# furiosa-ai/eta-inversion

Measured on AMD Instinct MI355X. Metric: images/sec SD1.5 512^2 50-step etainv+ptp, higher is better.
Workload: dtype bf16; 1 GPU; etainv+ptp, SD1.5-shaped UNet (seeded synthetic weights), 512x512 (64x64 latents), 50 DDIM steps, 32 image pairs per GPU per step, eta [[0.6, 0], [1, 0.7]], n=10 noise candidates, cfg 7.5/1; images_per_gpu=32, unet_sample_forwards_per_image_reference=300

## Files before the change

### eta-inversion_amd/csrc/common.h

```cpp
#pragma once
#include <hip/hip_runtime.h>
#include <stdint.h>
#include <stdio.h>
#include <stdlib.h>
#include <string>

#include "../../include/etainv.h"

namespace etainv {

typedef _Float16 f16;
typedef __bf16 bf16;
typedef float f32x4 __attribute__((ext_vector_type(4)));
typedef float f32x2 __attribute__((ext_vector_type(2)));
typedef float f32x16 __attribute__((ext_vector_type(16)));
typedef _Float16 f16x8 __attribute__((ext_vector_type(8)));
typedef _Float16 f16x4 __attribute__((ext_vector_type(4)));
typedef __bf16 bf16x8 __attribute__((ext_vector_type(8)));
typedef __bf16 bf16x4 __attribute__((ext_vector_type(4)));
typedef unsigned int u32x4 __attribute__((ext_vector_type(4)));
typedef unsigned int u32x2 __attribute__((ext_vector_type(2)));

void set_error(const std::string& msg);
#define ETAINV_FAIL(msg)                                                        \
// ... 16 lines not shown
    if (_e != hipSuccess) ETAINV_FAIL(std::string("launch: ") + hipGetErrorString(_e)); \
  } while (0)

template <typename T> __device__ __forceinline__ float to_f32(T v);
template <> __device__ __forceinline__ float to_f32<float>(float v) { return v; }
template <> __device__ __forceinline__ float to_f32<f16>(f16 v) { return (float)v; }
template <> __device__ __forceinline__ float to_f32<bf16>(bf16 v) { return (float)v; }
template <typename T> __device__ __forceinline__ T from_f32(float v);
template <> __device__ __forceinline__ float from_f32<float>(float v) { return v; }
template <> __device__ __forceinline__ f16 from_f32<f16>(float v) { return (f16)v; }
template <> __device__ __forceinline__ bf16 from_f32<bf16>(float v) { return (bf16)v; }

__device__ __forceinline__ float wave_sum(float v) {
#pragma unroll
  for (int o = 32; o > 0; o >>= 1) v += __shfl_xor(v, o, 64);
  return v;
}
__device__ __forceinline__ float wave_max(float v) {
#pragma unroll
  for (int o = 32; o > 0; o >>= 1) v = fmaxf(v, __shfl_xor(v, o, 64));
  return v;
}

__device__ __forceinline__ float silu_f(float x) { return x / (1.0f + __expf(-x)); }
typedef float gelu_f32x2 __attribute__((ext_vector_type(2)));
__device__ __forceinline__ gelu_f32x2 gelu_pair(gelu_f32x2 x) {
  gelu_f32x2 ax;
  ax[0] = fminf(fabsf(x[0]) * 0.70710678118654752f, 4.3f);
  ax[1] = fminf(fabsf(x[1]) * 0.70710678118654752f, 4.3f);
  gelu_f32x2 p = ax * 0.000100211372f + (-0.000461519738f);
  p = p * ax + (-0.00230234699f);
  p = p * ax + 0.0294526188f;
  p = p * ax + (-0.148963716f);
  p = p * ax + (-0.918328635f);
  p = p * ax + (-1.62791373f);
  const gelu_f32x2 t = p * ax;
  gelu_f32x2 e;
  e[0] = __builtin_amdgcn_exp2f(t[0]);
  e[1] = __builtin_amdgcn_exp2f(t[1]);
  const gelu_f32x2 er = 1.0f - e;
  gelu_f32x2 s;
  s[0] = copysignf(er[0], x[0]);
  s[1] = copysignf(er[1], x[1]);
  const gelu_f32x2 h = x * 0.5f;
  return h * s + h;
}
__device__ __forceinline__ float gelu_erf_f(float x) {
// ... 63 lines not shown
```

### eta-inversion_amd/csrc/kernels.h

```cpp
#pragma once
#include "common.h"

namespace etainv {

struct IGemmParams {
  const void* a1 = nullptr;
  const void* a2 = nullptr;
  const void* w = nullptr;
  const float* bias = nullptr;
  const float* rowvec = nullptr;
  int rowvec_stride = 0;
  int out_f32 = 0;
  int out_nchw = 0;
  int pad0 = 0;
  int out_io_dtype = 0;
  const void* residual = nullptr;
  void* out = nullptr;
  const void* zeros = nullptr;
  int debug = 0;
  int hm_heads = 0, hm_dim = 0, hm_tokens = 0, hm_magic = 0;
  unsigned long* stamps = nullptr;
  int M = 0, N = 0;
  int c1 = 0, c2 = 0;
  int H = 1, W = 1;
// ... 101 lines not shown
  float* maps_acc = nullptr;
  int xcd_gx = 0;
};
inline void cross_params_from_ctrl(CrossParams& cp, const etainv_attn_ctrl* ctrl) {
  if (!ctrl || (ctrl->mode != ETAINV_ATTN_PTP && ctrl->mode != ETAINV_ATTN_STORE)) return;
  const bool ptp = ctrl->mode == ETAINV_ATTN_PTP;
  cp.n_img = ctrl->n_img;
  cp.layout = ptp ? (ctrl->src_exit_block ? 3 : 2) : 1;
  cp.first_row = ptp ? ctrl->first_row : 0;
  if (ptp && (ctrl->mapper || ctrl->replace_mat)) {
    cp.edit = 1;
    cp.mapper = ctrl->mapper;
    cp.alphas = ctrl->alphas;
    cp.replace_mat = ctrl->replace_mat;
    cp.equalizer = ctrl->equalizer;
    cp.cross_alpha = ctrl->cross_alpha;
  }
}
int launch_cross_attention_p(const void* q, const void* kv, void* out, int b, int d, const CrossParams& p, int dtype, hipStream_t s);

int launch_im2col_in(const void* latent, int io_dtype, int n_lat, int rows, int L, void* out, int dtype, hipStream_t s);
int launch_time_embedding(const int64_t* t_host, int rows, int dim, void* out, int dtype, hipStream_t s);
int launch_silu(const void* x, void* out, int64_t n, int dtype, hipStream_t s);
enum PackMode { PK_PLAIN = 0, PK_CONV = 1, PK_GEGLU = 2, PK_CONV_IN_GEMM = 5 };
int launch_pack_ups4(const float* src, void* dst, int cout, int cin, int dtype, hipStream_t s);
int launch_pack_weight(const float* src, void* dst, int64_t rows, int64_t cols, int mode, int taps, int dtype, hipStream_t s, float scale = 1.0f,
                       const float* colscale = nullptr);
int launch_ln_fold(const float* w_src, const float* gamma, const float* beta, const float* bias_packed, int64_t rows, int64_t cols, int mode, float scale,
                   void* w_dst, float* s_dst, float* c_dst, int dtype, hipStream_t s);
int launch_cast_f32(const void* src, int src_dtype, void* dst, int dst_dtype, int64_t n, hipStream_t s);
int launch_rows_broadcast(void* x, int rows, int n_src, int64_t row_elems, int dtype, hipStream_t s);

int launch_prox_guidance(const float* eps_u, const float* eps_c, float g, int mode, int use_rank, int rank_lo, float rank_w, float thr_fixed,
                         float* eps_out, const float* x, float a_from, float a_to, float* x_out, float* thr_out, int n_groups, int rows_per_group,
                         int l, hipStream_t s);

int launch_image_metrics(const float* pred, const float* target, int b, int h, int w, float lo, float hi, int mask, float* out, void* workspace,
                         int64_t workspace_bytes, hipStream_t s);

int launch_word_maps(const float* maps_acc, int n_layers, int n_img_cap, int rows_per_img, int row_sel, int heads, int res, int L,
                     int n_img, const int32_t* tokens, int n_tok, int steps_done, float* out, int accumulate, float scale,
                     hipStream_t s, unsigned layer_mask = ~0u);
int launch_local_blend(const float* maps_acc, int n_layers, int n_img_cap, int heads, int res, int L, float* x, int n_img,
                       const float* blend_alpha, float thres, hipStream_t s);

}
// ... 1 lines not shown
```

### eta-inversion_amd/csrc/misc.hip

```cpp
#include <algorithm>

#include "common.h"
#include "kernels.h"

namespace etainv {

template <typename T, typename TIO>
__global__ void im2col_in_kernel(const TIO* __restrict__ x, int n_lat, int L, int rows, T* __restrict__ out) {
  const int LL = L * L;
  const int64_t i = (int64_t)blockIdx.x * blockDim.x + threadIdx.x;
  if (i >= (int64_t)rows * LL) return;
  const int row = (int)(i / LL), pix = (int)(i - (int64_t)row * LL);
  const int oy = pix / L, ox = pix - oy * L;
  const TIO* xb = x + (int64_t)(row % n_lat) * 4 * LL;
  T v[64];
#pragma unroll
  for (int k = 0; k < 64; ++k) v[k] = (T)0.f;
#pragma unroll
  for (int t = 0; t < 9; ++t) {
    const int iy = oy + t / 3 - 1, ix = ox + t % 3 - 1;
    if (iy >= 0 && iy < L && ix >= 0 && ix < L) {
#pragma unroll
      for (int ci = 0; ci < 4; ++ci) v[t * 4 + ci] = from_f32<T>(to_f32(xb[(int64_t)ci * LL + iy * L + ix]));
    }
  }
  u32x4* o = reinterpret_cast<u32x4*>(out + i * 64);
#pragma unroll
  for (int q = 0; q < (int)(64 * sizeof(T) / 16); ++q) o[q] = reinterpret_cast<u32x4*>(v)[q];
}

struct TimeVec { float t[64]; };
template <typename T>
__global__ void time_embedding_kernel(TimeVec tv, int uniform, int row0, int rows, int dim, T* __restrict__ out) {
  const int i = blockIdx.x * blockDim.x + threadIdx.x;
  if (i >= rows * dim) return;
  const int r = i / dim, c = i - r * dim, half = dim / 2;
  const int k = c < half ? c : c - half;
  const float freq = expf(-9.210340371976184f * (float)k / (float)half);
  const float a = tv.t[uniform ? 0 : r] * freq;
  out[(int64_t)row0 * dim + i] = from_f32<T>(c < half ? cosf(a) : sinf(a));
}

template <typename T>
__global__ void silu_kernel(const T* x, T* out, int64_t n) {
  int64_t i = (int64_t)blockIdx.x * blockDim.x + threadIdx.x;
  if (i < n) out[i] = from_f32<T>(silu_f(to_f32(x[i])));
}

template <typename TD>
__global__ void pack_weight_kernel(const float* __restrict__ src, TD* __restrict__ dst, int64_t rows, int64_t cols, int mode, int taps, float scale,
                                   const float* __restrict__ colscale) {
  const int64_t i = (int64_t)blockIdx.x * blockDim.x + threadIdx.x;
  if (mode == 5) {
    if (i >= rows * 64) return;
    const int64_t o = i / 64, k = i - o * 64, tap = k / 4, ci = k - tap * 4;
    dst[i] = from_f32<TD>(k < 36 ? src[o * 36 + ci * 9 + tap] : 0.f);
    return;
  }
  if (i >= rows * cols) return;
  int64_t s = i;
  if (mode == 1) {
    const int64_t o = i / cols, r = i - o * cols, cin = cols / taps;
    const int64_t t = r / cin, ci = r - t * cin;
    s = o * cols + ci * taps + t;
  } else if (mode == 2) {
    const int64_t p = i / cols, c = i - p * cols;
    const int64_t blk = p / 64, within = p % 64;
    const int64_t logical = within < 32 ? blk * 32 + within : rows / 2 + blk * 32 + within - 32;
    s = logical * cols + c;
// ... 47 lines not shown
}

int launch_time_embedding(const int64_t* t_host, int rows, int dim, void* out, int dtype, hipStream_t s) {
  ETAINV_CHECK(t_host && out && dim % 2 == 0 && rows > 0, "bad arguments");
  bool uniform = true;
  for (int i = 1; i < rows; ++i) uniform = uniform && t_host[i] == t_host[0];
  TimeVec tv;
  if (uniform) {
    tv.t[0] = (float)t_host[0];
    ETAINV_DISPATCH_DTYPE(dtype, T, hipLaunchKernelGGL(time_embedding_kernel<T>, dim3(cdiv(rows * dim, 256)), dim3(256), 0, s, tv, 1, 0, rows, dim, (T*)out));
  } else {
    for (int r0 = 0; r0 < rows; r0 += 64) {
      const int n = std::min(64, rows - r0);
      for (int i = 0; i < n; ++i) tv.t[i] = (float)t_host[r0 + i];
      ETAINV_DISPATCH_DTYPE(dtype, T, hipLaunchKernelGGL(time_embedding_kernel<T>, dim3(cdiv(n * dim, 256)), dim3(256), 0, s, tv, 0, r0, n, dim, (T*)out));
    }
  }
  ETAINV_LAUNCH_CHECK();
  return 0;
}

int launch_silu(const void* x, void* out, int64_t n, int dtype, hipStream_t s) {
  ETAINV_DISPATCH_DTYPE(dtype, T, hipLaunchKernelGGL(silu_kernel<T>, dim3(cdiv(n, 256)), dim3(256), 0, s, (const T*)x, (T*)out, n));
  ETAINV_LAUNCH_CHECK();
  return 0;
}

template <typename TD>
__global__ void pack_ups4_kernel(const float* __restrict__ src, TD* __restrict__ dst, int cout, int cin) {
  const int64_t total = (int64_t)16 * cout * cin;
  const int64_t i = (int64_t)blockIdx.x * 256 + threadIdx.x;
  if (i >= total) return;
  const int c = (int)(i % cin);
  const int t = (int)((i / cin) & 3);
  const int n = (int)((i / ((int64_t)4 * cin)) % cout);
  const int ph = (int)(i / ((int64_t)4 * cin * cout));
  const int py = ph >> 1, px = ph & 1, ty = t >> 1, tx = t & 1;
  const int ky0 = py == 0 ? (ty == 0 ? 0 : 1) : (ty == 0 ? 0 : 2), ky1 = py == 0 ? (ty == 0 ? 0 : 2) : (ty == 0 ? 1 : 2);
  const int kx0 = px == 0 ? (tx == 0 ? 0 : 1) : (tx == 0 ? 0 : 2), kx1 = px == 0 ? (tx == 0 ? 0 : 2) : (tx == 0 ? 1 : 2);
  const float* w = src + ((int64_t)n * cin + c) * 9;
  float v = 0.f;
  for (int ky = ky0; ky <= ky1; ++ky)
    for (int kx = kx0; kx <= kx1; ++kx) v += w[ky * 3 + kx];
  dst[i] = from_f32<TD>(v);
}
int launch_pack_ups4(const float* src, void* dst, int cout, int cin, int dtype, hipStream_t s) {
// ... 96 lines not shown
```

### eta-inversion_amd/csrc/norm.hip

```cpp
#include "common.h"
#include "kernels.h"

namespace etainv {

constexpr int GN_MAX_VEC_PER_LANE = 5;
#ifndef GN_UNROLL
#define GN_UNROLL 4
#endif

template <typename T> struct Vec8;
template <> struct Vec8<f16> { typedef f16x8 type; };
template <> struct Vec8<bf16> { typedef bf16x8 type; };

template <typename T>
__device__ __forceinline__ void load8(const T* p, float (&v)[8]) {
  typename Vec8<T>::type r = *reinterpret_cast<const typename Vec8<T>::type*>(p);
#pragma unroll
  for (int j = 0; j < 8; ++j) v[j] = (float)r[j];
}
template <typename T>
__device__ __forceinline__ void store8(T* p, const float (&v)[8]) {
  typename Vec8<T>::type r;
#pragma unroll
  for (int j = 0; j < 8; ++j) r[j] = (T)v[j];
// ... 55 lines not shown
    for (int o = 1; o < 8; o <<= 1) {
      a += __shfl_xor(a, o);
      c += __shfl_xor(c, o);
    }
    if (g < groups && sub == 0) {
      float* p = partial + (((int64_t)b * chunks + blockIdx.x) * groups + g) * 2;
      p[0] = a;
      p[1] = c;
    }
  } else if (threadIdx.x < groups) {
    const int g = threadIdx.x;
    float a = 0.f, c = 0.f;
    for (int w = 0; w < 4; ++w)
      for (int ch = g * cpg; ch < (g + 1) * cpg; ++ch) {
        a += sm[(w * C + ch) * 2 + 0];
        c += sm[(w * C + ch) * 2 + 1];
      }
    float* p = partial + (((int64_t)b * chunks + blockIdx.x) * groups + g) * 2;
    p[0] = a;
    p[1] = c;
  }
}

template <typename T, int VPL>
__global__ void __launch_bounds__(256) gn_apply_kernel(const T* __restrict__ x1, const T* __restrict__ x2, int c1, int c2, int hw,
                                                       int groups, const float* __restrict__ partial, int chunks_st, float count,
                                                       float eps, const float* __restrict__ gamma, const float* __restrict__ beta,
                                                       int silu, T* __restrict__ out) {
  const int C = c1 + c2, nvec = C >> 3, nv1 = c1 >> 3, cpg = C / groups;
  const int b = blockIdx.y, chunks = gridDim.x;
  const int per = (hw + chunks - 1) / chunks;
  const int beg = blockIdx.x * per, end = min(hw, beg + per);
  const int lane = threadIdx.x & 63, wid = threadIdx.x >> 6;
  __shared__ double s_red[8][64][2];
  __shared__ float st[64 * 2];
  const bool pre_scsh = chunks_st == 0 && gamma == nullptr;
  if (pre_scsh) {
  } else if (chunks_st == 0) {
    if (threadIdx.x < groups) {
      st[threadIdx.x * 2 + 0] = partial[((int64_t)b * groups + threadIdx.x) * 2 + 0];
      st[threadIdx.x * 2 + 1] = partial[((int64_t)b * groups + threadIdx.x) * 2 + 1];
    }
    __syncthreads();
  } else {
    const int NS = groups <= 32 ? 8 : 4;
    const int g = groups <= 32 ? (threadIdx.x & 31) : lane, slice = groups <= 32 ? (threadIdx.x >> 5) : wid;
    double a = 0.0, c = 0.0;
    if (g < groups) {
      f32x2 v[8];
#pragma unroll
      for (int u = 0; u < 8; ++u) {
        const int k = slice + u * NS;
        v[u] = (f32x2){0.f, 0.f};
        if (k < chunks_st) v[u] = *reinterpret_cast<const f32x2*>(partial + (((int64_t)b * chunks_st + k) * groups + g) * 2);
      }
#pragma unroll
      for (int u = 0; u < 8; ++u) { a += v[u][0]; c += v[u][1]; }
      for (int k = slice + 8 * NS; k < chunks_st; k += NS) {
        const float* p = partial + (((int64_t)b * chunks_st + k) * groups + g) * 2;
        a += p[0];
        c += p[1];
      }
      s_red[slice][g][0] = a;
      s_red[slice][g][1] = c;
    }
    __syncthreads();
    if (threadIdx.x < groups) {
      const int g = threadIdx.x;
      double sa = 0.0, sq = 0.0;
      for (int w = 0; w < NS; ++w) { sa += s_red[w][g][0]; sq += s_red[w][g][1]; }
      const double mean = sa / count;
      double var = sq / count - mean * mean;
      if (var < 0.0) var = 0.0;
      st[g * 2 + 0] = (float)mean;
      st[g * 2 + 1] = (float)(1.0 / sqrt(var + (double)eps));
    }
    __syncthreads();
  }
  if constexpr (VPL == 0) {
    constexpr int R = 5;
    const int G = 320 / nvec;
    float sc[R][8], sh[R][8];
    int poff[R], voff[R];
    bool second[R];
#pragma unroll
    for (int r = 0; r < R; ++r) {
      const int idx = lane + 64 * r;
      const int px = idx / nvec, v = idx - px * nvec;
      poff[r] = px;
      second[r] = v >= nv1;
      voff[r] = (second[r] ? v - nv1 : v) * 8;
      if (pre_scsh) {
        const float* ps = partial + ((int64_t)b * 2) * C + v * 8;
        *reinterpret_cast<f32x4*>(&sc[r][0]) = *reinterpret_cast<const f32x4*>(ps);
        *reinterpret_cast<f32x4*>(&sc[r][4]) = *reinterpret_cast<const f32x4*>(ps + 4);
        *reinterpret_cast<f32x4*>(&sh[r][0]) = *reinterpret_cast<const f32x4*>(ps + C);
        *reinterpret_cast<f32x4*>(&sh[r][4]) = *reinterpret_cast<const f32x4*>(ps + C + 4);
        continue;
      }
      int g = (v * 8) / cpg, rem = v * 8 - g * cpg;
#pragma unroll
      for (int j = 0; j < 8; ++j) {
        const int ch = v * 8 + j;
        const float a = st[g * 2 + 1] * gamma[ch];
        sc[r][j] = a;
        sh[r][j] = beta[ch] - st[g * 2] * a;
        if (++rem == cpg) { rem = 0; ++g; }
      }
    }
    for (int pix0 = beg + wid * G; pix0 < end; pix0 += 4 * G) {
      float t[R][8];
      bool ok[R];
#pragma unroll
      for (int r = 0; r < R; ++r) {
        const int pix = pix0 + poff[r];
        ok[r] = pix < end;
        const int64_t row = (int64_t)b * hw + (ok[r] ? pix : beg);
        if (second[r]) load8(x2 + row * c2 + voff[r], t[r]);
        else load8(x1 + row * c1 + voff[r], t[r]);
      }
#pragma unroll
      for (int r = 0; r < R; ++r) {
#pragma unroll
        for (int j = 0; j < 8; ++j) {
          const float y = t[r][j] * sc[r][j] + sh[r][j];
          t[r][j] = silu ? silu_f(y) : y;
        }
        const int pix = pix0 + poff[r];
        if (ok[r]) store8(out + ((int64_t)b * hw + pix) * C + (second[r] ? nv1 * 8 : 0) + voff[r], t[r]);
      }
    }
    return;
  }
  constexpr int VP = VPL > 0 ? VPL : 1;
  float sc[VP][8], sh[VP][8];
#pragma unroll
  for (int i = 0; i < VP; ++i) {
    const int v = lane + 64 * i;
    if (v < nvec) {
      if (pre_scsh) {
        const float* ps = partial + ((int64_t)b * 2) * C + v * 8;
        *reinterpret_cast<f32x4*>(&sc[i][0]) = *reinterpret_cast<const f32x4*>(ps);
        *reinterpret_cast<f32x4*>(&sc[i][4]) = *reinterpret_cast<const f32x4*>(ps + 4);
        *reinterpret_cast<f32x4*>(&sh[i][0]) = *reinterpret_cast<const f32x4*>(ps + C);
        *reinterpret_cast<f32x4*>(&sh[i][4]) = *reinterpret_cast<const f32x4*>(ps + C + 4);
        continue;
      }
      int g = (v * 8) / cpg, rem = v * 8 - g * cpg;
#pragma unroll
      for (int j = 0; j < 8; ++j) {
        const int ch = v * 8 + j;
        const float a = st[g * 2 + 1] * gamma[ch];
        sc[i][j] = a;
        sh[i][j] = beta[ch] - st[g * 2] * a;
        if (++rem == cpg) { rem = 0; ++g; }
      }
    }
  }
#pragma unroll(VP <= 2 ? GN_UNROLL : 1)
  for (int pix = beg + wid; pix < end; pix += 4) {
    const int64_t row = (int64_t)b * hw + pix;
#pragma unroll
    for (int i = 0; i < VP; ++i) {
      const int v = lane + 64 * i;
      if (v < nvec) {
        float t[8];
        if (v < nv1) load8(x1 + row * c1 + v * 8, t);
        else load8(x2 + row * c2 + (v - nv1) * 8, t);
#pragma unroll
        for (int j = 0; j < 8; ++j) {
          const float y = t[j] * sc[i][j] + sh[i][j];
          t[j] = silu ? silu_f(y) : y;
        }
        store8(out + row * C + v * 8, t);
      }
    }
  }
}

template <typename T>
__global__ void __launch_bounds__(256) layernorm_kernel(const T* __restrict__ x, const float* __restrict__ gamma,
                                                        const float* __restrict__ beta, T* __restrict__ out, int rows, int C,
                                                        float eps) {
  const int lane = threadIdx.x & 63;
  const int row = blockIdx.x * 4 + (threadIdx.x >> 6);
  if (row >= rows) return;
  const int nvec = C >> 3;
  float t[3][8];
  float sum = 0.f;
#pragma unroll
  for (int i = 0; i < 3; ++i) {
    const int v = lane + 64 * i;
    if (v < nvec) {
      load8(x + (int64_t)row * C + v * 8, t[i]);
#pragma unroll
      for (int j = 0; j < 8; ++j) sum += t[i][j];
    }
  }
  const float mean = wave_sum(sum) / (float)C;
// ... 94 lines not shown
  }
#pragma unroll
  for (int o = 1; o < 64; o <<= 1) {
    a += __shfl_xor(a, o);
    q += __shfl_xor(q, o);
  }
  const double count = (double)hw * (double)cpg;
  const double mean = a / count;
  double var = q / count - mean * mean;
  if (var < 0.0) var = 0.0;
  const float fmean = (float)mean, frstd = (float)(1.0 / sqrt(var + (double)eps));
  if (lane == 0) {
    final_stats[((int64_t)b * groups + g) * 2 + 0] = fmean;
    final_stats[((int64_t)b * groups + g) * 2 + 1] = frstd;
  }
  if (scsh)
    for (int ch = lo + lane; ch < hi; ch += 64) {
      const float sc = frstd * gamma[ch];
      scsh[((int64_t)b * 2 + 0) * C + ch] = sc;
      scsh[((int64_t)b * 2 + 1) * C + ch] = beta[ch] - fmean * sc;
    }
}

static inline int gn_apply_blocks() {
  static const int n = env_int("ETAINV_GN_APPLY_BLOCKS", 2048);
  return n;
}

static inline int gn_apply_mode(int C) {
  static const bool no_flat = env_on("ETAINV_GN_NOFLAT");
  const int nvec = C >> 3;
  if (!no_flat && (nvec == 40 || nvec == 80)) return 0;
  return (nvec + 63) / 64;
}

int launch_groupnorm(const void* x1, const void* x2, int c1, int c2, const float* gamma, const float* beta, void* out, int b,
                     int hw, int groups, float eps, int silu, float* scratch, int dtype, hipStream_t s) {
  if (dtype == ETAINV_F32) return launch_groupnorm_f32(x1, x2, c1, c2, gamma, beta, out, b, hw, groups, eps, silu, scratch, s);
  const int C = c1 + c2;
  ETAINV_CHECK(x1 && gamma && beta && out && scratch, "null pointer");
  ETAINV_CHECK(c1 % 8 == 0 && c2 % 8 == 0 && C % groups == 0 && groups <= 64, "channel layout");
  ETAINV_CHECK((C >> 3) <= 64 * GN_MAX_VEC_PER_LANE, "C too large");
  ETAINV_CHECK(c2 == 0 || x2, "second source missing");
  int chunks = std::min(GN_MAX_CHUNKS, std::max(1, std::min(hw / 8, 1024 / std::max(1, b))));
  float* partial = scratch;
  const size_t lds = (size_t)4 * C * 2 * sizeof(float);
  const int chunks_apply = std::max(1, std::min(hw / 4, std::max(chunks, gn_apply_blocks() / std::max(1, b))));
  ProfScope prof(PROF_GROUPNORM, 2.0 * 2.0 * (double)b * hw * C, s);
  const int vpl = ((C >> 3) + 63) / 64;
#define ETAINV_GN_LAUNCH(VPL_)                                                                                                             \
  {                                                                                                                                        \
    allow_dynamic_lds<&gn_stats_kernel<T, VPL_>>(4 * 64 * VPL_ * 8 * 2 * 4);                                                               \
    hipLaunchKernelGGL((gn_stats_kernel<T, VPL_>), dim3(chunks, b), dim3(256), lds, s, (const T*)x1, (const T*)x2, c1, c2, hw, groups, partial); \
  }
#define ETAINV_GN_APPLY(VPL_)                                                                                                              \
  hipLaunchKernelGGL((gn_apply_kernel<T, VPL_>), dim3(chunks_apply, b), dim3(256), 0, s, (const T*)x1, (const T*)x2, c1, c2, hw, groups,     \
                     (const float*)partial, chunks, (float)hw * (float)(C / groups), eps, gamma, beta, silu, (T*)out);
  ETAINV_DISPATCH_HALF(dtype, T, switch (vpl) {
    case 1: ETAINV_GN_LAUNCH(1) break;
    case 2: ETAINV_GN_LAUNCH(2) break;
    case 3: ETAINV_GN_LAUNCH(3) break;
    case 4: ETAINV_GN_LAUNCH(4) break;
    default: ETAINV_GN_LAUNCH(5) break;
  } switch (gn_apply_mode(C)) {
    case 0: ETAINV_GN_APPLY(0) break;
    case 1: ETAINV_GN_APPLY(1) break;
    case 2: ETAINV_GN_APPLY(2) break;
    case 3: ETAINV_GN_APPLY(3) break;
    case 4: ETAINV_GN_APPLY(4) break;
    default: ETAINV_GN_APPLY(5) break;
  });
#undef ETAINV_GN_APPLY
#undef ETAINV_GN_LAUNCH
  ETAINV_LAUNCH_CHECK();
  return 0;
}

int launch_gn_finalize(int c1, int c2, const float* part1, int wm1, const float* part2, int wm2, int b, int hw, int groups, float eps, float* final_stats,
                       hipStream_t s, const float* gamma, const float* beta, float* scsh) {
  ETAINV_CHECK(part1 && final_stats && (c1 + c2) % groups == 0 && groups <= 32, "bad arguments");
  ETAINV_CHECK(wm1 > 0 && hw % wm1 == 0 && (c2 == 0 || (part2 && wm2 > 0 && hw % wm2 == 0)), "row blocks must tile an image");
  ProfScope prof(PROF_GROUPNORM, 0.0, s);
  hipLaunchKernelGGL(gn_finalize_kernel, dim3((groups + 3) / 4, b), dim3(256), 0, s, part1, wm1, c1, part2, wm2, c2, hw, groups, eps, final_stats, gamma, beta,
                     scsh);
  ETAINV_LAUNCH_CHECK();
  return 0;
}

int launch_groupnorm_pre(const void* x1, const void* x2, int c1, int c2, const float* part1, int wm1, const float* part2, int wm2, const float* gamma,
                         const float* beta, void* out, int b, int hw, int groups, float eps, int silu, float* final_stats, int dtype, hipStream_t s) {
  const int C = c1 + c2;
  ETAINV_CHECK(x1 && gamma && beta && out && part1 && final_stats, "null pointer");
  ETAINV_CHECK(c1 % 8 == 0 && c2 % 8 == 0 && C % groups == 0 && groups <= 32, "channel layout");
  ETAINV_CHECK((C >> 3) <= 64 * GN_MAX_VEC_PER_LANE, "C too large");
  ETAINV_CHECK(c2 == 0 || (x2 && part2), "second source missing");
  ETAINV_CHECK(wm1 > 0 && hw % wm1 == 0 && (c2 == 0 || (wm2 > 0 && hw % wm2 == 0)), "row blocks must tile an image");
  ProfScope prof(PROF_GROUPNORM, 2.0 * 2.0 * (double)b * hw * C, s);
  prof_pause(true);
  float* scsh = final_stats + (int64_t)b * groups * 2;
  const int rc = launch_gn_finalize(c1, c2, part1, wm1, part2, wm2, b, hw, groups, eps, final_stats, s, gamma, beta, scsh);
  prof_pause(false);
  if (rc) return 1;
  const int chunks_apply = std::max(1, std::min(hw / 4, std::max(std::min(GN_MAX_CHUNKS, std::max(1, std::min(hw / 8, 1024 / std::max(1, b)))), gn_apply_blocks() / std::max(1, b))));
#define ETAINV_GN_APPLY(VPL_)                                                                                                              \
  hipLaunchKernelGGL((gn_apply_kernel<T, VPL_>), dim3(chunks_apply, b), dim3(256), 0, s, (const T*)x1, (const T*)x2, c1, c2, hw, groups,     \
                     (const float*)scsh, 0, (float)hw * (float)(C / groups), eps, (const float*)nullptr, (const float*)nullptr, silu, (T*)out);
  ETAINV_DISPATCH_HALF(dtype, T, switch (gn_apply_mode(C)) {
    case 0: ETAINV_GN_APPLY(0) break;
    case 1: ETAINV_GN_APPLY(1) break;
    case 2: ETAINV_GN_APPLY(2) break;
    case 3: ETAINV_GN_APPLY(3) break;
    case 4: ETAINV_GN_APPLY(4) break;
    default: ETAINV_GN_APPLY(5) break;
  });
#undef ETAINV_GN_APPLY
  ETAINV_LAUNCH_CHECK();
  return 0;
}

int launch_layernorm(const void* x, const float* gamma, const float* beta, void* out, int rows, int c, float eps, int dtype,
                     hipStream_t s) {
  if (dtype == ETAINV_F32) return launch_layernorm_f32(x, gamma, beta, out, rows, c, eps, s);
  ETAINV_CHECK(x && gamma && beta && out, "null pointer");
  ETAINV_CHECK(c % 8 == 0 && (c >> 3) <= 192, "LayerNorm width must be a multiple of 8 and <= 1536");
  ProfScope prof(PROF_LAYERNORM, 2.0 * 2.0 * (double)rows * c, s);
  ETAINV_DISPATCH_HALF(dtype, T,
                       hipLaunchKernelGGL(layernorm_kernel<T>, dim3(cdiv(rows, 4)), dim3(256), 0, s, (const T*)x, gamma, beta,
                                          (T*)out, rows, c, eps));
  ETAINV_LAUNCH_CHECK();
  return 0;
}

int launch_row_stats(const void* x, float* stat, int rows, int c, float eps, int dtype, hipStream_t s) {
  ETAINV_CHECK(x && stat, "null pointer");
  ETAINV_CHECK(c % 8 == 0 && (c >> 3) <= 192, "row width must be a multiple of 8 and <= 1536");
  ProfScope prof(PROF_LAYERNORM, 2.0 * (double)rows * c, s);
  ETAINV_DISPATCH_HALF(dtype, T, hipLaunchKernelGGL(row_stats_kernel<T>, dim3(cdiv(rows, 4)), dim3(256), 0, s, (const T*)x, stat, rows, c, eps));
// ... 14 lines not shown
```

### eta-inversion_amd/csrc/ops_capi.cpp

```cpp
#include <cmath>

#include "common.h"
#include "kernels.h"

using namespace etainv;

extern "C" int etainv_op_gemm(const void* a, const void* w, const void* bias, const void* residual, void* out, int m, int n, int k,
                              int geglu, int dtype, void* stream) {
  IGemmParams p = igemm_linear(a, w, (const float*)bias, out, m, n, k);
  p.residual = residual;
  p.geglu = geglu;
  return launch_igemm(p, dtype, (hipStream_t)stream);
}

extern "C" int etainv_op_gemm_ln(const void* a, const void* w_folded, const float* c_vec, const float* s_vec, const float* stat,
                                 const void* residual, void* out, float* stat_out, int* stat_p_out, int m, int n, int k, int geglu,
                                 int dtype, void* stream) {
  IGemmParams p = igemm_linear(a, w_folded, c_vec, out, m, n, k);
  p.residual = residual;
  p.geglu = geglu;
  if (stat) {
    p.ln_stat = stat;
    p.ln_s = s_vec;
  }
// ... 150 lines not shown
}

extern "C" int etainv_op_gemm_per_image(const void* a, const void* wb, const float* cb, const void* residual, void* out, int b, int hw, int n, int k,
                                        int dtype, void* stream) {
  ETAINV_CHECK(b > 0 && hw > 0, "bad sizes");
  IGemmParams p = igemm_linear(a, wb, cb, out, b * hw, n, k);
  p.residual = residual;
  p.rows_per_batch = hw;
  p.w_batch_stride = (int64_t)n * k;
  p.bias_batch_stride = n;
  return launch_igemm(p, dtype, (hipStream_t)stream);
}

extern "C" int etainv_op_time_embedding(const int64_t* t_host, int rows, int dim, void* out, int dtype, void* stream) {
  return launch_time_embedding(t_host, rows, dim, out, dtype, (hipStream_t)stream);
}

extern "C" int etainv_op_silu(const void* x, void* out, int64_t n, int dtype, void* stream) {
  ETAINV_CHECK(x && out && n >= 0, "null pointer or negative size");
  if (n == 0) return 0;
  return launch_silu(x, out, n, dtype, (hipStream_t)stream);
}

extern "C" int etainv_op_cast(const void* src, int src_dtype, void* dst, int dst_dtype, int64_t n, void* stream) {
  ETAINV_CHECK(src && dst && n >= 0, "null pointer or negative size");
  if (n == 0) return 0;
  return launch_cast_f32(src, src_dtype, dst, dst_dtype, n, (hipStream_t)stream);
}

extern "C" int etainv_op_im2col_in(const void* latent, int io_dtype, int n_lat, int rows, int l, void* out, int dtype, void* stream) {
  ETAINV_CHECK(l > 0, "bad sizes");
  return launch_im2col_in(latent, io_dtype, n_lat, rows, l, out, dtype, (hipStream_t)stream);
}

extern "C" int etainv_op_pack_weight(const float* src, void* dst, int64_t rows, int64_t cols, int mode, int taps, float scale, const float* colscale,
                                     int dtype, void* stream) {
  return launch_pack_weight(src, dst, rows, cols, mode, taps, dtype, (hipStream_t)stream, scale, colscale);
}

extern "C" int etainv_op_word_maps_ex(const float* maps_acc, int n_layers, int n_img_cap, int heads, int res, int L, int n_img, const int32_t* tokens,
                                      int n_tok, int steps_done, int row_sel, unsigned layer_mask, float* out, int accumulate, float scale, void* stream) {
  ETAINV_CHECK(row_sel == 0 || row_sel == 1, "row_sel: 0 = source cond row, 1 = target cond row");
  ETAINV_CHECK(n_img <= n_img_cap && heads > 0 && res > 0 && L > 0, "bad sizes");
  return launch_word_maps(maps_acc, n_layers, n_img_cap, 2, row_sel, heads, res, L, n_img, tokens, n_tok, steps_done, out, accumulate, scale,
                          (hipStream_t)stream, layer_mask);
}
// ... 13 lines not shown
```

### eta-inversion_amd/etainv/_capi.py

```python
import ctypes as C
import os
from pathlib import Path

F32, F16, BF16 = 0, 1, 2
ATTN_PLAIN, ATTN_STORE, ATTN_PTP, ATTN_MASA, ATTN_PNP = 0, 1, 2, 3, 4

_LIB_PATH = Path(__file__).resolve().parent / "lib" / "libetainv_hip.so"


class EtainvError(RuntimeError):
    pass


class EngineConfig(C.Structure):
    _fields_ = [("compute_dtype", C.c_int), ("max_unet_batch", C.c_int), ("latent_size", C.c_int), ("max_img", C.c_int),
                ("reserved", C.c_int * 4)]


class AttnCtrl(C.Structure):
    _fields_ = [("mode", C.c_int), ("n_img", C.c_int), ("store_maps", C.c_int),
                ("mapper", C.c_void_p), ("alphas", C.c_void_p), ("replace_mat", C.c_void_p), ("equalizer", C.c_void_p),
                ("cross_alpha", C.c_void_p),
                ("self_replace_active", C.c_int), ("self_max_tokens", C.c_int),
                ("masa_active", C.c_int), ("masa_first_block", C.c_int), ("first_row", C.c_int), ("src_exit_block", C.c_int), ("pnp_qk_active", C.c_int), ("pnp_conv_active", C.c_int)]
# ... 51 lines not shown
    "etainv_op_conv3x3_gnstat": [_p, _p, _p, _p, _p, _p, _p, C.POINTER(_i), _i, _i, _i, _i, _i, _i, _p],
    "etainv_op_groupnorm_pre": [_p, _p, _i, _i, _p, _i, _p, _i, _p, _p, _p, _i, _i, _i, _f, _i, _p, _i, _p],
    "etainv_op_ln_fold": [_p, _p, _p, _p, _i, _i, _i, _f, _p, _p, _p, _i, _p],
    "etainv_op_row_stats": [_p, _p, _i, _i, _f, _i, _p],
    "etainv_op_ln_finalize": [_p, _i, _i, _f, _p, _i, _p],
    "etainv_op_pack_ups4": [_p, _p, _i, _i, _i, _p],
    "etainv_op_conv3x3": [_p, _p, _i, _i, _p, _p, _p, _p, _p, _i, _i, _i, _i, _i, _i, _i, _i, _p],
    "etainv_op_conv3x3_ex": [_p, _p, _p, _p, _p, _i, _i, _i, _i, _i, _i, _i, _i, _i, _i, _i, _p],
    "etainv_op_im2col3x3": [_p, _i, _i, _i, _i, _i, _p, _p, _i, _p],
    "etainv_op_row_softmax": [_p, _i, _i, _f, _i, _p],
    "etainv_op_quick_gelu": [_p, _p, _i64, _i, _p],
    "etainv_op_embed": [_p, _p, _p, _i, _i, _i, _p, _i, _p],
    "etainv_op_causal_attention": [_p, _p, _i, _i, _i, _i, _i, _p],
    "etainv_op_groupnorm": [_p, _p, _i, _i, _p, _p, _p, _i, _i, _i, _f, _i, _p, _i, _p],
    "etainv_op_layernorm": [_p, _p, _p, _p, _i, _i, _f, _i, _p],
    "etainv_op_self_attention": [_p, _p, _i, _i, _i, _i, _i, _i, _i, _p],
    "etainv_op_self_attention_ex": [_p, _p, _i, _i, _i, _i, _i, _i, _i, _i, _i, _i, _p],
    "etainv_op_cross_attention": [_p, _p, _p, _i, _i, _i, _i, _i, C.POINTER(AttnCtrl), _i, _i, _p, _i, _p],
    "etainv_op_word_maps": [_p, _i, _i, _i, _i, _i, _i, _p, _i, _i, _p, _i, _f, _p],
    "etainv_op_local_blend": [_p, _i, _i, _i, _i, _i, _p, _i, _p, _f, _p],
    "etainv_op_word_maps_ex": [_p, _i, _i, _i, _i, _i, _i, _p, _i, _i, _i, C.c_uint, _p, _i, _f, _p],
    "etainv_op_time_embedding": [C.POINTER(_i64), _i, _i, _p, _i, _p],
    "etainv_op_silu": [_p, _p, _i64, _i, _p],
    "etainv_op_cast": [_p, _i, _p, _i, _i64, _p],
    "etainv_op_im2col_in": [_p, _i, _i, _i, _i, _p, _i, _p],
    "etainv_op_pack_weight": [_p, _p, _i64, _i64, _i, _i, _f, _p, _i, _p],
    "etainv_op_gemm_f32out": [_p, _p, _p, _p, _i, _i, _i, _i, _p],
    "etainv_op_conv3x3_rv": [_p, _p, _i, _i, _p, _p, _p, _i, _p, _p, _i, _i, _i, _i, _i, _i, _i, _i, _p],
    "etainv_op_gn_fold": [_p, _p, _p, _p, _p, _i, _i, _i, _i, _p, _p, _i, _p],
    "etainv_op_gemm_per_image": [_p, _p, _p, _p, _p, _i, _i, _i, _i, _i, _p],
    "etainv_op_rows_broadcast": [_p, _i, _i, _i64, _i, _p],
}
_RESTYPES = {"etainv_last_error": C.c_char_p, "etainv_engine_workspace_bytes": _i64, "etainv_image_metrics_workspace_bytes": _i64, "etainv_engine_weight_bytes": _i64}

_lib = None


def lib_path() -> Path:
    return Path(os.environ.get("ETAINV_LIB", _LIB_PATH))


def load():
    global _lib
    if _lib is None:
        path = lib_path()
        if not path.exists():
# ... 31 lines not shown
```

### include/etainv.h

```cpp
#ifndef ETAINV_H
#define ETAINV_H
#include <stdint.h>
#ifdef __cplusplus
extern "C" {
#endif

#define ETAINV_ABI_VERSION 1
#define ETAINV_MAX_WORDS 77

enum etainv_dtype { ETAINV_F32 = 0, ETAINV_F16 = 1, ETAINV_BF16 = 2 };

int etainv_abi_version(void);
const char* etainv_last_error(void);


int etainv_cfg_combine(const void* eps_u, const void* eps_c, float g, void* out, int64_t n,
                       int io_dtype, void* stream);

int etainv_ddim_step(const void* x, const void* eps, float a_from, float a_to, void* out, int64_t n,
                     int io_dtype, void* stream);

int etainv_ddim_eta_step(const void* x, const void* eps, float eta, const void* eta_mask, int n_mask, const void* noise,
                         float a_t, float a_p, float var, int rows, int c, int hw, void* out, int io_dtype, void* stream);

// ... 140 lines not shown
int etainv_op_groupnorm(const void* x_nhwc, const void* x2_nhwc, int c1, int c2, const float* gamma,
                        const float* beta, void* out, int b, int hw, int groups, float eps, int silu,
                        float* scratch, int dtype, void* stream);
int etainv_op_layernorm(const void* x, const float* gamma, const float* beta, void* out, int rows, int c,
                        float eps, int dtype, void* stream);
int etainv_op_self_attention(const void* qkv, void* out, int b, int n, int heads, int d, int mode, int n_img,
                             int dtype, void* stream);
int etainv_op_self_attention_ex(const void* qkv, void* out, int b, int n, int heads, int d, int mode, int n_img,
                                int q_prescaled, int first_row, int head_major, int dtype, void* stream);
int etainv_op_cross_attention(const void* q, const void* kv, void* out, int b, int n, int heads, int d,
                              int n_ctx, const etainv_attn_ctrl* ctrl, int map_layer, int n_img_cap,
                              float* maps_acc, int dtype, void* stream);
int etainv_op_word_maps(const float* maps_acc, int n_layers, int n_img_cap, int heads, int res, int L, int n_img,
                        const int32_t* tokens, int n_tok, int steps_done, float* out, int accumulate, float scale,
                        void* stream);
int etainv_op_local_blend(const float* maps_acc, int n_layers, int n_img_cap, int heads, int res, int L, float* x,
                          int n_img, const float* blend_alpha, float thres, void* stream);

int etainv_op_word_maps_ex(const float* maps_acc, int n_layers, int n_img_cap, int heads, int res, int L, int n_img,
                           const int32_t* tokens, int n_tok, int steps_done, int row_sel, unsigned layer_mask, float* out,
                           int accumulate, float scale, void* stream);
int etainv_op_time_embedding(const int64_t* t_host, int rows, int dim, void* out, int dtype, void* stream);
int etainv_op_silu(const void* x, void* out, int64_t n, int dtype, void* stream);
int etainv_op_cast(const void* src, int src_dtype, void* dst, int dst_dtype, int64_t n, void* stream);
int etainv_op_im2col_in(const void* latent, int io_dtype, int n_lat, int rows, int l, void* out, int dtype, void* stream);
int etainv_op_pack_weight(const float* src, void* dst, int64_t rows, int64_t cols, int mode, int taps, float scale, const float* colscale,
                          int dtype, void* stream);
int etainv_op_rows_broadcast(void* x, int rows, int n_src, int64_t row_elems, int dtype, void* stream);
int etainv_op_gemm_f32out(const void* a, const void* w, const float* bias, float* out_f32, int m, int n, int k, int dtype, void* stream);
int etainv_op_conv3x3_rv(const void* x_nhwc, const void* x2_nhwc, int c1, int c2, const void* w_okkc, const void* bias,
                         const float* rowvec, int rowvec_stride, const void* residual, void* out, int b, int h, int wd, int cout,
                         int stride, int upsample, int taps, int dtype, void* stream);
int etainv_op_gn_fold(const float* w, const float* gamma, const float* beta, const float* bias, const float* stats, int groups, int b, int n,
                      int k, void* wb_out, float* cb_out, int dtype, void* stream);
int etainv_op_gemm_per_image(const void* a, const void* wb, const float* cb, const void* residual, void* out, int b, int hw, int n, int k,
                             int dtype, void* stream);

#ifdef __cplusplus
}
#endif
#endif
```

Baseline: 5.866 images/s.

## Rewrite GroupNorm apply kernel with fast SiLU, prefetch pipeline and 320-thread blocks

Replaces the multi-mode GroupNorm apply kernel with one templated kernel: each thread owns one 8-channel vector, uses 320-thread blocks sized to the channel count, and prefetches the next group of four rows while computing the current one. SiLU now uses a reciprocal plus one Newton correction instead of a true division, and falls back to the exact division only when an input is in a rare range. A sweep kernel is added to check that the fast SiLU matches the division bit-for-bit. The intent is lower ALU cost and better memory latency hiding in the GroupNorm+SiLU passes, at the cost of losing the earlier per-width specialisations and their environment tuning knobs.

```diff
diff --git a/eta-inversion_amd/csrc/common.h b/eta-inversion_amd/csrc/common.h
--- a/eta-inversion_amd/csrc/common.h
+++ b/eta-inversion_amd/csrc/common.h
@@ -62,7 +62,19 @@
   return v;
 }
 
-__device__ __forceinline__ float silu_f(float x) { return x / (1.0f + __expf(-x)); }
+__device__ __forceinline__ float silu_div_f(float x) { return x / (1.0f + __expf(-x)); }
+__device__ __forceinline__ float silu_fast_f(float x) {
+  const float d = 1.0f + __expf(-x);
+  const float r = __builtin_amdgcn_rcpf(d);
+  const float q = x * r;
+  return fmaf(fmaf(-q, d, x), r, q);
+}
+__device__ __forceinline__ uint32_t silu_range_key(float x) { return (__float_as_uint(x) & 0x7fffffffu) - 1u; }
+__device__ __forceinline__ bool silu_key_is_rare(uint32_t key) { return key >= 0x42ae0000u; }
+__device__ __forceinline__ float silu_f(float x) {
+  if (__builtin_expect(silu_key_is_rare(silu_range_key(x)), 0)) return silu_div_f(x);
+  return silu_fast_f(x);
+}
 typedef float gelu_f32x2 __attribute__((ext_vector_type(2)));
 __device__ __forceinline__ gelu_f32x2 gelu_pair(gelu_f32x2 x) {
   gelu_f32x2 ax;
diff --git a/eta-inversion_amd/csrc/kernels.h b/eta-inversion_amd/csrc/kernels.h
--- a/eta-inversion_amd/csrc/kernels.h
+++ b/eta-inversion_amd/csrc/kernels.h
@@ -147,6 +147,7 @@
 int launch_im2col_in(const void* latent, int io_dtype, int n_lat, int rows, int L, void* out, int dtype, hipStream_t s);
 int launch_time_embedding(const int64_t* t_host, int rows, int dim, void* out, int dtype, hipStream_t s);
 int launch_silu(const void* x, void* out, int64_t n, int dtype, hipStream_t s);
+int launch_silu_sweep(uint32_t first, uint64_t count, uint64_t* mismatches, uint32_t* first_bad, hipStream_t s);
 enum PackMode { PK_PLAIN = 0, PK_CONV = 1, PK_GEGLU = 2, PK_CONV_IN_GEMM = 5 };
 int launch_pack_ups4(const float* src, void* dst, int cout, int cin, int dtype, hipStream_t s);
 int launch_pack_weight(const float* src, void* dst, int64_t rows, int64_t cols, int mode, int taps, int dtype, hipStream_t s, float scale = 1.0f,
diff --git a/eta-inversion_amd/csrc/misc.hip b/eta-inversion_amd/csrc/misc.hip
--- a/eta-inversion_amd/csrc/misc.hip
+++ b/eta-inversion_amd/csrc/misc.hip
@@ -45,6 +45,25 @@
 __global__ void silu_kernel(const T* x, T* out, int64_t n) {
   int64_t i = (int64_t)blockIdx.x * blockDim.x + threadIdx.x;
   if (i < n) out[i] = from_f32<T>(silu_f(to_f32(x[i])));
+}
+
+__global__ void silu_sweep_kernel(uint32_t first, uint64_t count, unsigned long long* mismatches, uint32_t* first_bad) {
+  const uint64_t stride = (uint64_t)gridDim.x * blockDim.x;
+  unsigned long long bad = 0;
+  uint32_t lowest = 0xffffffffu;
+  for (uint64_t i = (uint64_t)blockIdx.x * blockDim.x + threadIdx.x; i < count; i += stride) {
+    const uint32_t bits = first + (uint32_t)i;
+    const float x = __uint_as_float(bits);
+    const float a = silu_f(x), d = silu_div_f(x);
+    if (!(__float_as_uint(a) == __float_as_uint(d) || (a != a && d != d))) {
+      ++bad;
+      lowest = min(lowest, bits);
+    }
+  }
+  if (bad) {
+    atomicAdd(mismatches, bad);
+    atomicMin(first_bad, lowest);
+  }
 }
 
 template <typename TD>
@@ -138,6 +157,17 @@
 
 int launch_silu(const void* x, void* out, int64_t n, int dtype, hipStream_t s) {
   ETAINV_DISPATCH_DTYPE(dtype, T, hipLaunchKernelGGL(silu_kernel<T>, dim3(cdiv(n, 256)), dim3(256), 0, s, (const T*)x, (T*)out, n));
+  ETAINV_LAUNCH_CHECK();
+  return 0;
+}
+
+int launch_silu_sweep(uint32_t first, uint64_t count, uint64_t* mismatches, uint32_t* first_bad, hipStream_t s) {
+  ETAINV_CHECK(mismatches && first_bad && count <= (1ull << 32), "null pointer or more than 2^32 patterns");
+  ETAINV_HIP(hipMemsetAsync(mismatches, 0, sizeof(uint64_t), s));
+  ETAINV_HIP(hipMemsetAsync(first_bad, 0xff, sizeof(uint32_t), s));
+  if (count == 0) return 0;
+  const int blocks = (int)std::min<uint64_t>((count + 255) / 256, 256 * 32);
+  hipLaunchKernelGGL(silu_sweep_kernel, dim3(blocks), dim3(256), 0, s, first, count, (unsigned long long*)mismatches, first_bad);
   ETAINV_LAUNCH_CHECK();
   return 0;
 }
diff --git a/eta-inversion_amd/csrc/norm.hip b/eta-inversion_amd/csrc/norm.hip
--- a/eta-inversion_amd/csrc/norm.hip
+++ b/eta-inversion_amd/csrc/norm.hip
@@ -101,51 +101,57 @@
   }
 }
 
-template <typename T, int VPL>
-__global__ void __launch_bounds__(256) gn_apply_kernel(const T* __restrict__ x1, const T* __restrict__ x2, int c1, int c2, int hw,
-                                                       int groups, const float* __restrict__ partial, int chunks_st, float count,
-                                                       float eps, const float* __restrict__ gamma, const float* __restrict__ beta,
-                                                       int silu, T* __restrict__ out) {
+constexpr int GN_APPLY_U = 4;
+constexpr int GN_APPLY_THREADS = 320;
+
+template <typename T, bool SILU>
+__global__ void __launch_bounds__(GN_APPLY_THREADS) gn_apply_kernel(const T* __restrict__ x1, const T* __restrict__ x2, int c1, int c2, int hw,
+                                                                    int groups, const float* __restrict__ partial, int chunks_st, float count,
+                                                                    float eps, const float* __restrict__ gamma, const float* __restrict__ beta,
+                                                                    T* __restrict__ out) {
+  typedef typename Vec8<T>::type V8;
+  constexpr int U = GN_APPLY_U;
   const int C = c1 + c2, nvec = C >> 3, nv1 = c1 >> 3, cpg = C / groups;
   const int b = blockIdx.y, chunks = gridDim.x;
-  const int per = (hw + chunks - 1) / chunks;
-  const int beg = blockIdx.x * per, end = min(hw, beg + per);
-  const int lane = threadIdx.x & 63, wid = threadIdx.x >> 6;
+  const int beg = (int)((int64_t)hw * blockIdx.x / chunks), end = (int)((int64_t)hw * (blockIdx.x + 1) / chunks);
+  const int tid = threadIdx.x;
   __shared__ double s_red[8][64][2];
   __shared__ float st[64 * 2];
   const bool pre_scsh = chunks_st == 0 && gamma == nullptr;
   if (pre_scsh) {
   } else if (chunks_st == 0) {
-    if (threadIdx.x < groups) {
-      st[threadIdx.x * 2 + 0] = partial[((int64_t)b * groups + threadIdx.x) * 2 + 0];
-      st[threadIdx.x * 2 + 1] = partial[((int64_t)b * groups + threadIdx.x) * 2 + 1];
+    if (tid < groups) {
+      st[tid * 2 + 0] = partial[((int64_t)b * groups + tid) * 2 + 0];
+      st[tid * 2 + 1] = partial[((int64_t)b * groups + tid) * 2 + 1];
     }
     __syncthreads();
   } else {
     const int NS = groups <= 32 ? 8 : 4;
-    const int g = groups <= 32 ? (threadIdx.x & 31) : lane, slice = groups <= 32 ? (threadIdx.x >> 5) : wid;
-    double a = 0.0, c = 0.0;
-    if (g < groups) {
-      f32x2 v[8];
-#pragma unroll
-      for (int u = 0; u < 8; ++u) {
-        const int k = slice + u * NS;
-        v[u] = (f32x2){0.f, 0.f};
-        if (k < chunks_st) v[u] = *reinterpret_cast<const f32x2*>(partial + (((int64_t)b * chunks_st + k) * groups + g) * 2);
+    for (int item = tid; item < 256; item += blockDim.x) {
+      const int g = groups <= 32 ? (item & 31) : (item & 63), slice = groups <= 32 ? (item >> 5) : (item >> 6);
+      double a = 0.0, c = 0.0;
+      if (g < groups) {
+        f32x2 v[8];
+#pragma unroll
+        for (int u = 0; u < 8; ++u) {
+          const int k = slice + u * NS;
+          v[u] = (f32x2){0.f, 0.f};
+          if (k < chunks_st) v[u] = *reinterpret_cast<const f32x2*>(partial + (((int64_t)b * chunks_st + k) * groups + g) * 2);
+        }
+#pragma unroll
+        for (int u = 0; u < 8; ++u) { a += v[u][0]; c += v[u][1]; }
+        for (int k = slice + 8 * NS; k < chunks_st; k += NS) {
+          const float* p = partial + (((int64_t)b * chunks_st + k) * groups + g) * 2;
+          a += p[0];
+          c += p[1];
+        }
+        s_red[slice][g][0] = a;
+        s_red[slice][g][1] = c;
       }
-#pragma unroll
-      for (int u = 0; u < 8; ++u) { a += v[u][0]; c += v[u][1]; }
-      for (int k = slice + 8 * NS; k < chunks_st; k += NS) {
-        const float* p = partial + (((int64_t)b * chunks_st + k) * groups + g) * 2;
-        a += p[0];
-        c += p[1];
-      }
-      s_red[slice][g][0] = a;
-      s_red[slice][g][1] = c;
     }
     __syncthreads();
-    if (threadIdx.x < groups) {
-      const int g = threadIdx.x;
+    if (tid < groups) {
+      const int g = tid;
       double sa = 0.0, sq = 0.0;
       for (int w = 0; w < NS; ++w) { sa += s_red[w][g][0]; sq += s_red[w][g][1]; }
       const double mean = sa / count;
@@ -156,104 +162,73 @@
     }
     __syncthreads();
   }
-  if constexpr (VPL == 0) {
-    constexpr int R = 5;
-    const int G = 320 / nvec;
-    float sc[R][8], sh[R][8];
-    int poff[R], voff[R];
-    bool second[R];
-#pragma unroll
-    for (int r = 0; r < R; ++r) {
-      const int idx = lane + 64 * r;
-      const int px = idx / nvec, v = idx - px * nvec;
-      poff[r] = px;
-      second[r] = v >= nv1;
-      voff[r] = (second[r] ? v - nv1 : v) * 8;
-      if (pre_scsh) {
-        const float* ps = partial + ((int64_t)b * 2) * C + v * 8;
-        *reinterpret_cast<f32x4*>(&sc[r][0]) = *reinterpret_cast<const f32x4*>(ps);
-        *reinterpret_cast<f32x4*>(&sc[r][4]) = *reinterpret_cast<const f32x4*>(ps + 4);
-        *reinterpret_cast<f32x4*>(&sh[r][0]) = *reinterpret_cast<const f32x4*>(ps + C);
-        *reinterpret_cast<f32x4*>(&sh[r][4]) = *reinterpret_cast<const f32x4*>(ps + C + 4);
-        continue;
+  const int pl = tid / nvec, v = tid - pl * nvec, ppb = blockDim.x / nvec;
+  float sc[8], sh[8];
+  if (pre_scsh) {
+    const float* ps = partial + ((int64_t)b * 2) * C + v * 8;
+    *reinterpret_cast<f32x4*>(&sc[0]) = *reinterpret_cast<const f32x4*>(ps);
+    *reinterpret_cast<f32x4*>(&sc[4]) = *reinterpret_cast<const f32x4*>(ps + 4);
+    *reinterpret_cast<f32x4*>(&sh[0]) = *reinterpret_cast<const f32x4*>(ps + C);
+    *reinterpret_cast<f32x4*>(&sh[4]) = *reinterpret_cast<const f32x4*>(ps + C + 4);
+  } else {
+    int g = (v * 8) / cpg, rem = v * 8 - g * cpg;
+#pragma unroll
+    for (int j = 0; j < 8; ++j) {
+      const int ch = v * 8 + j;
+      const float a = st[g * 2 + 1] * gamma[ch];
+      sc[j] = a;
+      sh[j] = beta[ch] - st[g * 2] * a;
+      if (++rem == cpg) { rem = 0; ++g; }
+    }
+  }
+  const bool second = v >= nv1;
+  const int cs = second ? c2 : c1;
+  const T* src = (second ? x2 + (v - nv1) * 8 : x1 + v * 8) + ((int64_t)b * hw + beg) * cs;
+  const T* const safe = src;
+  T* dst = out + ((int64_t)b * hw + beg) * C + v * 8;
+  const int64_t sstep = (int64_t)ppb * cs, dstep = (int64_t)ppb * C;
+  src += (int64_t)pl * cs;
+  dst += (int64_t)pl * C;
+  int left = end - beg - pl;
+  if (left <= 0) return;
+  auto normalise = [&](const V8& raw) {
+    V8 o;
+    float y[8];
+    uint32_t key = 0;
+#pragma unroll
+    for (int j = 0; j < 8; ++j) {
+      y[j] = fmaf((float)raw[j], sc[j], sh[j]);
+      if (SILU) {
+        o[j] = (T)silu_fast_f(y[j]);
+        key = max(key, silu_range_key(y[j]));
+      } else {
+        o[j] = (T)y[j];
       }
-      int g = (v * 8) / cpg, rem = v * 8 - g * cpg;
-#pragma unroll
-      for (int j = 0; j < 8; ++j) {
-        const int ch = v * 8 + j;
-        const float a = st[g * 2 + 1] * gamma[ch];
-        sc[r][j] = a;
-        sh[r][j] = beta[ch] - st[g * 2] * a;
-        if (++rem == cpg) { rem = 0; ++g; }
-      }
-    }
-    for (int pix0 = beg + wid * G; pix0 < end; pix0 += 4 * G) {
-      float t[R][8];
-      bool ok[R];
-#pragma unroll
-      for (int r = 0; r < R; ++r) {
-        const int pix = pix0 + poff[r];
-        ok[r] = pix < end;
-        const int64_t row = (int64_t)b * hw + (ok[r] ? pix : beg);
-        if (second[r]) load8(x2 + row * c2 + voff[r], t[r]);
-        else load8(x1 + row * c1 + voff[r], t[r]);
-      }
-#pragma unroll
-      for (int r = 0; r < R; ++r) {
-#pragma unroll
-        for (int j = 0; j < 8; ++j) {
-          const float y = t[r][j] * sc[r][j] + sh[r][j];
-          t[r][j] = silu ? silu_f(y) : y;
-        }
-        const int pix = pix0 + poff[r];
-        if (ok[r]) store8(out + ((int64_t)b * hw + pix) * C + (second[r] ? nv1 * 8 : 0) + voff[r], t[r]);
-      }
-    }
-    return;
-  }
-  constexpr int VP = VPL > 0 ? VPL : 1;
-  float sc[VP][8], sh[VP][8];
-#pragma unroll
-  for (int i = 0; i < VP; ++i) {
-    const int v = lane + 64 * i;
-    if (v < nvec) {
-      if (pre_scsh) {
-        const float* ps = partial + ((int64_t)b * 2) * C + v * 8;
-        *reinterpret_cast<f32x4*>(&sc[i][0]) = *reinterpret_cast<const f32x4*>(ps);
-        *reinterpret_cast<f32x4*>(&sc[i][4]) = *reinterpret_cast<const f32x4*>(ps + 4);
-        *reinterpret_cast<f32x4*>(&sh[i][0]) = *reinterpret_cast<const f32x4*>(ps + C);
-        *reinterpret_cast<f32x4*>(&sh[i][4]) = *reinterpret_cast<const f32x4*>(ps + C + 4);
-        continue;
-      }
-      int g = (v * 8) / cpg, rem = v * 8 - g * cpg;
-#pragma unroll
-      for (int j = 0; j < 8; ++j) {
-        const int ch = v * 8 + j;
-        const float a = st[g * 2 + 1] * gamma[ch];
-        sc[i][j] = a;
-        sh[i][j] = beta[ch] - st[g * 2] * a;
-        if (++rem == cpg) { rem = 0; ++g; }
-      }
-    }
-  }
-#pragma unroll(VP <= 2 ? GN_UNROLL : 1)
-  for (int pix = beg + wid; pix < end; pix += 4) {
-    const int64_t row = (int64_t)b * hw + pix;
-#pragma unroll
-    for (int i = 0; i < VP; ++i) {
-      const int v = lane + 64 * i;
-      if (v < nvec) {
-        float t[8];
-        if (v < nv1) load8(x1 + row * c1 + v * 8, t);
-        else load8(x2 + row * c2 + (v - nv1) * 8, t);
-#pragma unroll
-        for (int j = 0; j < 8; ++j) {
-          const float y = t[j] * sc[i][j] + sh[i][j];
-          t[j] = silu ? silu_f(y) : y;
-        }
-        store8(out + row * C + v * 8, t);
-      }
-    }
+    }
+    if (SILU && __builtin_expect(silu_key_is_rare(key), 0)) {
+#pragma unroll
+      for (int j = 0; j < 8; ++j) o[j] = (T)silu_div_f(y[j]);
+    }
+    return o;
+  };
+  V8 nxt[U];
+#pragma unroll
+  for (int u = 0; u < U; ++u) nxt[u] = *reinterpret_cast<const V8*>(u * ppb < left ? src + u * sstep : safe);
+  for (; left > 0; left -= U * ppb) {
+    V8 cur[U];
+#pragma unroll
+    for (int u = 0; u < U; ++u) cur[u] = nxt[u];
+    src += U * sstep;
+    if (left > U * ppb) {
+#pragma unroll
+      for (int u = 0; u < U; ++u) nxt[u] = *reinterpret_cast<const V8*>((U + u) * ppb < left ? src + u * sstep : safe);
+    }
+#pragma unroll
+    for (int u = 0; u < U; ++u) {
+      const V8 o = normalise(cur[u]);
+      if (u * ppb < left) *reinterpret_cast<V8*>(dst + u * dstep) = o;
+    }
+    dst += U * dstep;
   }
 }
 
@@ -394,16 +369,15 @@
     }
 }
 
-static inline int gn_apply_blocks() {
-  static const int n = env_int("ETAINV_GN_APPLY_BLOCKS", 2048);
-  return n;
-}
-
-static inline int gn_apply_mode(int C) {
-  static const bool no_flat = env_on("ETAINV_GN_NOFLAT");
-  const int nvec = C >> 3;
-  if (!no_flat && (nvec == 40 || nvec == 80)) return 0;
-  return (nvec + 63) / 64;
+template <typename T, bool SILU>
+static int gn_apply_launch(const T* x1, const T* x2, int c1, int c2, int hw, int groups, const float* partial, int chunks_st, float eps,
+                           const float* gamma, const float* beta, T* out, int b, hipStream_t s) {
+  const int C = c1 + c2, nvec = C >> 3, ppb = GN_APPLY_THREADS / nvec;
+  const int chunks_stats = std::min(GN_MAX_CHUNKS, std::max(1, std::min(hw / 8, 1024 / std::max(1, b))));
+  const int chunks = std::max(1, std::min(hw / 4, std::max(chunks_stats, 2048 / std::max(1, b))));
+  hipLaunchKernelGGL((gn_apply_kernel<T, SILU>), dim3(chunks, b), dim3(ppb * nvec), 0, s, x1, x2, c1, c2, hw, groups, partial, chunks_st,
+                     (float)hw * (float)(C / groups), eps, gamma, beta, out);
+  return 0;
 }
 
 int launch_groupnorm(const void* x1, const void* x2, int c1, int c2, const float* gamma, const float* beta, void* out, int b,
@@ -417,7 +391,6 @@
   int chunks = std::min(GN_MAX_CHUNKS, std::max(1, std::min(hw / 8, 1024 / std::max(1, b))));
   float* partial = scratch;
   const size_t lds = (size_t)4 * C * 2 * sizeof(float);
-  const int chunks_apply = std::max(1, std::min(hw / 4, std::max(chunks, gn_apply_blocks() / std::max(1, b))));
   ProfScope prof(PROF_GROUPNORM, 2.0 * 2.0 * (double)b * hw * C, s);
   const int vpl = ((C >> 3) + 63) / 64;
 #define ETAINV_GN_LAUNCH(VPL_)                                                                                                             \
@@ -425,23 +398,15 @@
     allow_dynamic_lds<&gn_stats_kernel<T, VPL_>>(4 * 64 * VPL_ * 8 * 2 * 4);                                                               \
     hipLaunchKernelGGL((gn_stats_kernel<T, VPL_>), dim3(chunks, b), dim3(256), lds, s, (const T*)x1, (const T*)x2, c1, c2, hw, groups, partial); \
   }
-#define ETAINV_GN_APPLY(VPL_)                                                                                                              \
-  hipLaunchKernelGGL((gn_apply_kernel<T, VPL_>), dim3(chunks_apply, b), dim3(256), 0, s, (const T*)x1, (const T*)x2, c1, c2, hw, groups,     \
-                     (const float*)partial, chunks, (float)hw * (float)(C / groups), eps, gamma, beta, silu, (T*)out);
+#define ETAINV_GN_APPLY(SILU_)                                                                                                             \
+  if (gn_apply_launch<T, SILU_>((const T*)x1, (const T*)x2, c1, c2, hw, groups, partial, chunks, eps, gamma, beta, (T*)out, b, s)) return 1;
   ETAINV_DISPATCH_HALF(dtype, T, switch (vpl) {
     case 1: ETAINV_GN_LAUNCH(1) break;
     case 2: ETAINV_GN_LAUNCH(2) break;
     case 3: ETAINV_GN_LAUNCH(3) break;
     case 4: ETAINV_GN_LAUNCH(4) break;
     default: ETAINV_GN_LAUNCH(5) break;
-  } switch (gn_apply_mode(C)) {
-    case 0: ETAINV_GN_APPLY(0) break;
-    case 1: ETAINV_GN_APPLY(1) break;
-    case 2: ETAINV_GN_APPLY(2) break;
-    case 3: ETAINV_GN_APPLY(3) break;
-    case 4: ETAINV_GN_APPLY(4) break;
-    default: ETAINV_GN_APPLY(5) break;
-  });
+  } if (silu) { ETAINV_GN_APPLY(true) } else { ETAINV_GN_APPLY(false) });
 #undef ETAINV_GN_APPLY
 #undef ETAINV_GN_LAUNCH
   ETAINV_LAUNCH_CHECK();
@@ -473,18 +438,9 @@
   const int rc = launch_gn_finalize(c1, c2, part1, wm1, part2, wm2, b, hw, groups, eps, final_stats, s, gamma, beta, scsh);
   prof_pause(false);
   if (rc) return 1;
-  const int chunks_apply = std::max(1, std::min(hw / 4, std::max(std::min(GN_MAX_CHUNKS, std::max(1, std::min(hw / 8, 1024 / std::max(1, b)))), gn_apply_blocks() / std::max(1, b))));
-#define ETAINV_GN_APPLY(VPL_)                                                                                                              \
-  hipLaunchKernelGGL((gn_apply_kernel<T, VPL_>), dim3(chunks_apply, b), dim3(256), 0, s, (const T*)x1, (const T*)x2, c1, c2, hw, groups,     \
-                     (const float*)scsh, 0, (float)hw * (float)(C / groups), eps, (const float*)nullptr, (const float*)nullptr, silu, (T*)out);
-  ETAINV_DISPATCH_HALF(dtype, T, switch (gn_apply_mode(C)) {
-    case 0: ETAINV_GN_APPLY(0) break;
-    case 1: ETAINV_GN_APPLY(1) break;
-    case 2: ETAINV_GN_APPLY(2) break;
-    case 3: ETAINV_GN_APPLY(3) break;
-    case 4: ETAINV_GN_APPLY(4) break;
-    default: ETAINV_GN_APPLY(5) break;
-  });
+#define ETAINV_GN_APPLY(SILU_)                                                                                                             \
+  if (gn_apply_launch<T, SILU_>((const T*)x1, (const T*)x2, c1, c2, hw, groups, scsh, 0, eps, nullptr, nullptr, (T*)out, b, s)) return 1;
+  ETAINV_DISPATCH_HALF(dtype, T, if (silu) { ETAINV_GN_APPLY(true) } else { ETAINV_GN_APPLY(false) });
 #undef ETAINV_GN_APPLY
   ETAINV_LAUNCH_CHECK();
   return 0;
diff --git a/eta-inversion_amd/csrc/ops_capi.cpp b/eta-inversion_amd/csrc/ops_capi.cpp
--- a/eta-inversion_amd/csrc/ops_capi.cpp
+++ b/eta-inversion_amd/csrc/ops_capi.cpp
@@ -196,6 +196,10 @@
   return launch_silu(x, out, n, dtype, (hipStream_t)stream);
 }
 
+extern "C" int etainv_op_silu_sweep(uint32_t first, uint64_t count, uint64_t* mismatches, uint32_t* first_bad, void* stream) {
+  return launch_silu_sweep(first, count, mismatches, first_bad, (hipStream_t)stream);
+}
+
 extern "C" int etainv_op_cast(const void* src, int src_dtype, void* dst, int dst_dtype, int64_t n, void* stream) {
   ETAINV_CHECK(src && dst && n >= 0, "null pointer or negative size");
   if (n == 0) return 0;
diff --git a/eta-inversion_amd/etainv/_capi.py b/eta-inversion_amd/etainv/_capi.py
--- a/eta-inversion_amd/etainv/_capi.py
+++ b/eta-inversion_amd/etainv/_capi.py
@@ -97,6 +97,7 @@
     "etainv_op_word_maps_ex": [_p, _i, _i, _i, _i, _i, _i, _p, _i, _i, _i, C.c_uint, _p, _i, _f, _p],
     "etainv_op_time_embedding": [C.POINTER(_i64), _i, _i, _p, _i, _p],
     "etainv_op_silu": [_p, _p, _i64, _i, _p],
+    "etainv_op_silu_sweep": [C.c_uint32, C.c_uint64, _p, _p, _p],
     "etainv_op_cast": [_p, _i, _p, _i, _i64, _p],
     "etainv_op_im2col_in": [_p, _i, _i, _i, _i, _p, _i, _p],
     "etainv_op_pack_weight": [_p, _p, _i64, _i64, _i, _i, _f, _p, _i, _p],
diff --git a/include/etainv.h b/include/etainv.h
--- a/include/etainv.h
+++ b/include/etainv.h
@@ -186,6 +186,7 @@
                            int accumulate, float scale, void* stream);
 int etainv_op_time_embedding(const int64_t* t_host, int rows, int dim, void* out, int dtype, void* stream);
 int etainv_op_silu(const void* x, void* out, int64_t n, int dtype, void* stream);
+int etainv_op_silu_sweep(uint32_t first, uint64_t count, uint64_t* mismatches, uint32_t* first_bad, void* stream);
 int etainv_op_cast(const void* src, int src_dtype, void* dst, int dst_dtype, int64_t n, void* stream);
 int etainv_op_im2col_in(const void* latent, int io_dtype, int n_lat, int rows, int l, void* out, int dtype, void* stream);
 int etainv_op_pack_weight(const float* src, void* dst, int64_t rows, int64_t cols, int mode, int taps, float scale, const float* colscale,
```

After: 5.889 images/s (median of 6 runs). Within noise of the previous version (+0.4%).
